# TrackieWay-OSS/TrackieLLM

Hardware: AMD Instinct MI355X
Metric: cortex cycles/sec (frame+1s audio+128 tok) (higher is better)
Workload: dtype int8 x q4_K/q6_K (i32 acc, f32 scales); 1 GPU; configs[3] fused cycle: YOLOv8n 640x640 frame (preprocess+network+NMS) + 1 s PCM (VAD + Whisper-tiny.en log-mel/encoder/16 forced decoder steps) + Mistral-7B Q4_K_M 64-token prefill and 128-token greedy decode, 3 concurrent HIP streams; concurrent_cycles_per_gpu=768, decode_groups=3, rows_per_llm_pass=256, layers=32, parallelism=replicas x1

## Files before the change

trackiellm_amd/csrc/audio/tk_audio_engine.h:

```cpp
#ifndef TK_AUDIO_ENGINE_H
#define TK_AUDIO_ENGINE_H

#include <hip/hip_runtime.h>
#include <stdint.h>

#include <string>
#include <vector>

#include "../common/tk_whisper_graph.h"

class TkWhisperModel {
public:
    TkWhisperHP hp{};
    TkWhManifest man;
    int device = 0;
    std::vector<float*> w;
    std::vector<uint8_t*> wt;
    bool prepare_tiles();
    int tensor_of(const float* dev_ptr) const;
    std::string error;
    ~TkWhisperModel();
    bool init(const TkWhisperHP& hp, int device);
    bool fill_synthetic(uint64_t seed);
    bool set_tensor(int idx, const float* host, size_t n);
    bool load_file(const char* path);
    bool load_ggml(class TkWhisperGgml& g);
};

class TkAsr {
public:
    TkWhisperModel* model = nullptr;
    int max_batch = 1;
    bool fast = false;
    std::string error;
    hipStream_t stream = nullptr;
    ~TkAsr();
    bool init(TkWhisperModel* m, int max_batch);
    bool transcribe(int B, const int16_t* pcm, int n_samples, const int32_t* prompt, int n_prompt, int n_steps, int32_t* tokens_out,
                    std::vector<float>* mel_out, std::vector<float>* enc_out, std::vector<float>* first_logits);
    bool transcribe_policy(int B, const int16_t* pcm, int n_samples, const int32_t* prompt, int n_prompt, int n_steps, float temperature, uint64_t seed,
                           int32_t* tokens_out, float* logprobs_out);
    bool transcribe_ref(int B, const int16_t* pcm, int n_samples, const int32_t* n_samples_row, const int32_t* prompt, int n_prompt, int n_steps, float temperature,
                        uint64_t seed, const uint8_t* suppress, int32_t token_beg, int32_t token_eot, int32_t* tokens_out, float* logprobs_out, int32_t* result_len,
                        int32_t* status);

private:
    friend struct TkAudioGpuOps;
    float* arena = nullptr;
    size_t arena_floats = 0, arena_used = 0;
    std::string launch_error;
    int16_t* pcm_dev = nullptr;
    size_t pcm_cap = 0;
    struct { bool on = false; float temp = 0.0f; uint64_t seed = 0; float* logprob = nullptr; int step = 0;
             bool filtered = false; int first_step = 0; const uint8_t* suppress = nullptr; int32_t* state = nullptr; int32_t beg = 0, eot = 0, tid0 = 0; } pick;
    uint8_t* suppress_dev = nullptr;
    std::vector<uint8_t> suppress_host;
    int32_t* wh_state = nullptr;
    float* lp_dev = nullptr;
    bool ensure_decode_buffers();
    std::vector<float> pick_logprobs;
};

class TkVadModel {
public:
    int device = 0, window = 480, hidden = 64;
    float *w1 = nullptr, *b1 = nullptr, *w2 = nullptr, *b2 = nullptr;
    float *x = nullptr, *hbuf = nullptr, *p = nullptr;
    int cap = 0;
    hipStream_t stream = nullptr;
    std::string error;
    ~TkVadModel();
    bool init(int device, int window, int hidden);
    bool fill_synthetic(uint64_t seed);
    bool infer(const float* windows_host, int n, float* prob_host);
};

#endif
```

trackiellm_amd/csrc/audio/tk_audio_engine.hip:

```cpp
#include "tk_audio_engine.h"
#include "tk_whisper_ggml.h"

#include <stdio.h>
#include <string.h>

#include "../nn/tk_gemm_tiled.h"
#include "../nn/tk_nn_kernels.h"

static inline hipError_t tk_create_perception_stream(hipStream_t* s) {
    int lo = 0, hi = 0;
    if (hipDeviceGetStreamPriorityRange(&lo, &hi) != hipSuccess) return hipStreamCreateWithFlags(s, hipStreamNonBlocking);
    return hipStreamCreateWithPriority(s, hipStreamNonBlocking, hi);
}

#define HIPQ(expr)                                                                              \
    do {                                                                                        \
        hipError_t e__ = (expr);                                                                \
        if (e__ != hipSuccess) {                                                                \
            char b__[256];                                                                      \
            snprintf(b__, sizeof b__, "%s failed: %s (%s:%d)", #expr, hipGetErrorString(e__), __FILE__, __LINE__); \
            error = b__;                                                                        \
            return false;                                                                       \
        }                                                                                       \
    } while (0)


__global__ void k_frames(const int16_t* pcm, int n_samples, int pcm_stride, int n_total, int T, const float* window, float* out) {
    const int b = blockIdx.z;
    const int64_t i = (int64_t)blockIdx.x * blockDim.x + threadIdx.x;
    if (i >= (int64_t)T * TK_WH_NFFT) return;
    const int t = (int)(i / TK_WH_NFFT), n = (int)(i % TK_WH_NFFT);
    int j = t * TK_WH_HOP + n - TK_WH_NFFT / 2;
    if (j < 0) j = -j;
    if (j >= n_total) j = 2 * (n_total - 1) - j;
    const float x = j < n_samples ? tk_divf((float)pcm[(int64_t)b * pcm_stride + j], 32768.0f) : 0.0f;
    out[((int64_t)b * T + t) * TK_WH_NFFT + n] = x * window[n];
}

__global__ void k_power(const float* ri, int64_t rows, int nb, float* out) {
    const int64_t i = (int64_t)blockIdx.x * blockDim.x + threadIdx.x;
    if (i >= rows * nb) return;
    const int64_t r = i / nb;
    const int f = (int)(i % nb);
    const float re = ri[r * 2 * nb + f], im = ri[r * 2 * nb + nb + f];
    out[i] = tk_fmaf(re, re, im * im);
}

__global__ __launch_bounds__(1024) void k_logmel_finish(float* mel, int per_b) {
    __shared__ float red[16];
    float* m = mel + (int64_t)blockIdx.x * per_b;
    float mx = -INFINITY;
    for (int i = threadIdx.x; i < per_b; i += 1024) {
        const float v = tk_log10f(tk_fmaxf(m[i], 1e-10f));
        m[i] = v;
        mx = tk_fmaxf(mx, v);
    }
    for (int s = 32; s >= 1; s >>= 1) mx = tk_fmaxf(mx, __shfl_xor(mx, s, 64));
    if ((threadIdx.x & 63) == 0) red[threadIdx.x >> 6] = mx;
    __syncthreads();
    mx = red[0];
    for (int w = 1; w < 16; ++w) mx = tk_fmaxf(mx, red[w]);
    const float floor_v = mx - 8.0f;
    for (int i = threadIdx.x; i < per_b; i += 1024) m[i] = (tk_fmaxf(m[i], floor_v) + 4.0f) * 0.25f;
}


#define TK_AT1_CK 64
#define TK_AT1_NS 3
__device__ __forceinline__ void at1_wait_vmcnt(int n) {
#define TK_VMW(k) case k: __builtin_amdgcn_s_waitcnt(0x0F70 | ((k) & 15) | (((k) >> 4) << 14)); break;
    switch (n) {
        TK_VMW(0) TK_VMW(1) TK_VMW(2) TK_VMW(3) TK_VMW(4) TK_VMW(5) TK_VMW(6) TK_VMW(7) TK_VMW(8) TK_VMW(9) TK_VMW(10) TK_VMW(11) TK_VMW(12)
        TK_VMW(13) TK_VMW(14) TK_VMW(15) TK_VMW(16)
        default: __builtin_amdgcn_s_waitcnt(0x0F70); break;
    }
#undef TK_VMW
}
__global__ __launch_bounds__(256) void k_attend1(const float* q, const float* k, const float* v, float* out, int Tk, int64_t q_bstride, int64_t kv_bstride, int d,
                                                 int hd, float scale, float* img ) {
    extern __shared__ __attribute__((aligned(16))) float att1_lds[];
    __shared__ float red[4];
    float* vring = att1_lds;
    float* sc = att1_lds + (size_t)TK_AT1_NS * TK_AT1_CK * hd;
    float* qs = sc + Tk;
    const int h = blockIdx.x, b = blockIdx.y, t0 = threadIdx.x, lane = t0 & 63;
    const int wave = __builtin_amdgcn_readfirstlane(t0 >> 6);
// ... 118 lines not shown
    float* image_for(const float* A, int M, int K, int lda) {
        pk.mark = a->arena_used;
        TkGemm g{};
        g.M = M; g.K = K;
        pk.img = raw_alloc(tk_tiled_gemm_scratch(g));
        pk.A = A; pk.M = M; pk.K = K; pk.lda = lda; pk.live = true;
        return pk.img;
    }
    void gemm(const TkGemm& g) {
        if (a->fast && long_ok) {
            drop_image();
            TkGemm f = g;
            f.fast = 1;
            tk_launch_gemm(f, s);
            return;
        }
        const int idx = tk_tiled_gemm_applies(g) ? a->model->tensor_of(g.B) : -1;
        if (idx < 0 || !a->model->wt[(size_t)idx]) { drop_image(); tk_launch_gemm(g, s); return; }
        if (!(pk.live && pk.A == g.A && pk.M == g.M && pk.K == g.K && pk.lda == g.lda)) {
            drop_image();
            pk.mark = a->arena_used;
            pk.img = raw_alloc(tk_tiled_gemm_scratch(g));
            tk_launch_pack_a(g.A, g.M, g.K, g.lda, 0, pk.img, s);
            pk.A = g.A; pk.M = g.M; pk.K = g.K; pk.lda = g.lda; pk.live = true;
        }
        const float* c0 = g.C;
        const float* c1 = g.C + (size_t)(g.M - 1) * g.ldc + g.N;
        const float* a0 = g.A;
        const float* a1 = g.A + (size_t)(g.M - 1) * g.lda + g.K;
        const bool in_place = c0 < a1 && a0 < c1;
        const bool plain = !g.residual && !g.c_feeds_linear && g.N % 16 == 0 && !in_place;
        if (plain) {
            if (pend.n > 0 && (pend.t.a_img != pk.img || pend.t.K != g.K || pend.t.nrows != g.M || pend.t.act != g.act)) flush();
            TkTiledGemm& t = pend.t;
            if (pend.n == 0) {
                t = TkTiledGemm{};
                t.wbytes = 4; t.K = g.K; t.ks = 1; t.nrows = g.M; t.slab_rows = 0; t.a_img = pk.img; t.a_ts = (size_t)g.K * 16;
                t.act = g.act; t.add_zero_bias = 1; t.per_seg = 1;
            }
            const int i = pend.n++;
            t.tiles[i] = a->model->wt[(size_t)idx]; t.row_tiles[i] = g.N / 16;
            t.seg_out[i] = g.C; t.seg_ldc[i] = g.ldc; t.seg_bias[i] = g.bias; t.seg_n[i] = g.N;
            if (pend.n == 3) flush();
            return;
        }
        flush();
        TkTiledGemm t{};
        t.tiles[0] = a->model->wt[(size_t)idx]; t.row_tiles[0] = (g.N + 15) / 16; t.nseg = 1; t.wbytes = 4;
        t.K = g.K; t.ks = 1; t.ldc = g.ldc; t.n_valid = g.N; t.nrows = g.M; t.slab_rows = 0;
        t.a_img = pk.img; t.a_ts = (size_t)g.K * 16; t.out = g.C;
        t.bias = g.bias; t.residual = g.residual; t.ldr = g.ldr; t.act = g.act; t.add_zero_bias = 1;
        const bool emit_img = g.c_feeds_linear && g.N % 128 == 0 && g.ldc == g.N && !g.residual && !in_place;
        float* cimg = nullptr;
        if (emit_img) {
            TkGemm nx{};
            nx.M = g.M; nx.K = g.N;
            cimg = raw_alloc(tk_tiled_gemm_scratch(nx));
            t.c_img = cimg;
        }
        if (!tk_launch_gemm_tiled(t, s)) tk_launch_gemm(g, s);
        if (emit_img) {
            pk.img = cimg; pk.A = g.C; pk.M = g.M; pk.K = g.N; pk.lda = g.ldc; pk.live = true;
            return;
        }
        if (in_place) drop_image();
    }
    void im2col1d(const float* x, int B, int T, int C, int ldx, int kw, int stride, int pad, float* col) { drop_image(); tk_launch_im2col1d(x, B, T, C, ldx, kw, stride, pad, col, s); }
    void layernorm(const float* x, int rows, int D, const float* w, const float* b, float* y) {
        drop_image();
        float* img = D % 128 == 0 && !(a->fast && long_ok) ? image_for(y, rows, D, D) : nullptr;
        tk_launch_layernorm(x, rows, D, w, b, TK_WH_LN_EPS, y, s, img);
    }
    void softmax_rows(float* x, int rows, int cols, int ld) { drop_image(); tk_launch_softmax_rows(x, rows, cols, ld, s); }
    bool attend1(const float* q, const float* k, const float* v, float* out, int B, int Tk, int64_t q_bstride, int64_t kv_bstride, int d, int nh) {
        drop_image();
        const int hd = d / nh;
        const size_t ldsb = ((size_t)TK_AT1_NS * TK_AT1_CK * hd + (size_t)Tk + (size_t)hd) * 4;
        if (hd > 256 || (hd & 15) || (d & 3) || Tk < 1 || ldsb > 60 * 1024) return false;
        float* img = (short_pass(B) && d % 128 == 0 && q_bstride == d) ? image_for(out, B, d, d) : nullptr;
        hipLaunchKernelGGL(k_attend1, dim3(nh, B), dim3(256), ldsb, s, q, k, v, out, Tk, q_bstride, kv_bstride, d, hd, tk_divf(1.0f, tk_sqrtf((float)hd)), img);
        return true;
    }
    bool attend_fused(const float* q, const float* k, const float* v, float* out, int B, int Tq, int Tk, int64_t q_bstride, int64_t kv_bstride, int d, int nh) {
        if (!a->fast || !long_ok || Tq < 2 || nh < 1 || d != nh * 64) return false;
        drop_image();
        return tk_launch_attention_h3(q, k, v, out, B, nh, Tq, Tk, q_bstride, kv_bstride, d, tk_divf(1.0f, tk_sqrtf(64.0f)), s);
    }
    void add_rows(float* x, const float* add, int rows, int D, int add_rows) { drop_image(); tk_launch_add_rows(x, add, rows, D, add_rows, s); }
    void embed_rows(const float* table, const float* pos, const int32_t* idx, const int32_t* pos_idx, int rows, int D, float* out) {
        drop_image();
        tk_launch_embed_rows(table, pos, idx, pos_idx, rows, D, out, s);
    }
    void argmax_rows(const float* x, int rows, int cols, int ld, int32_t* out) {
        drop_image();
        if (!a->pick.on) { tk_launch_argmax_rows(x, rows, cols, ld, out, s); return; }
        TkPick pk{a->pick.temp, a->pick.seed, (uint32_t)(a->pick.step * rows), a->pick.logprob ? a->pick.logprob + (size_t)a->pick.step * rows : nullptr};
        if (a->pick.filtered) {
            if (a->pick.step >= a->pick.first_step) {
                TkWhFilter f{a->pick.suppress, a->pick.state, a->pick.beg, a->pick.eot, a->pick.tid0};
                tk_launch_pick_rows_filtered(x, rows, cols, ld, out, pk, f, s);
            }
        } else {
            tk_launch_pick_rows(x, rows, cols, ld, out, pk, s);
        }
        a->pick.step++;
    }
    void frames(const int16_t* pcm, int B, int n_samples, int pcm_stride, int n_total, int T, const float* window, float* out) {
        drop_image();
        const int64_t per = (int64_t)T * TK_WH_NFFT;
        hipLaunchKernelGGL(k_frames, dim3((unsigned)((per + 255) / 256), 1, B), dim3(256), 0, s, pcm, n_samples, pcm_stride, n_total, T, window, out);
    }
    void power(const float* ri, int rows, int nb, float* out) {
        drop_image();
        const int64_t n = (int64_t)rows * nb;
        hipLaunchKernelGGL(k_power, dim3((unsigned)((n + 255) / 256)), dim3(256), 0, s, ri, (int64_t)rows, nb, out);
    }
    void logmel_finish(float* mel, int B, int per_b) { drop_image(); hipLaunchKernelGGL(k_logmel_finish, dim3(B), dim3(1024), 0, s, mel, per_b); }
};

struct TkAudioSizeOps {
    size_t used = 0, peak = 0;
    float* alloc(size_t n) { used += (n + 63) & ~(size_t)63; if (used > peak) peak = used; return nullptr; }
    int32_t* alloc_i32(size_t n) { return (int32_t*)alloc(n); }
    void gemm(const TkGemm& g) {
        if (!tk_tiled_gemm_applies(g)) return;
        size_t top = used + ((tk_tiled_gemm_scratch(g) + 63) & ~(size_t)63);
        if (g.c_feeds_linear) { TkGemm nx{}; nx.M = g.M; nx.K = g.N; top += (tk_tiled_gemm_scratch(nx) + 63) & ~(size_t)63; }
        if (top > peak) peak = top;
    }
    void image(int M, int K) {
        TkGemm g{};
        g.M = M; g.K = K;
        const size_t top = used + ((tk_tiled_gemm_scratch(g) + 63) & ~(size_t)63);
        if (top > peak) peak = top;
    }
    void im2col1d(const float*, int, int, int, int, int, int, int, float*) {}
    void layernorm(const float*, int rows, int D, const float*, const float*, float*) { image(rows, D); }
    void softmax_rows(float*, int, int, int) {}
    bool attend1(const float*, const float*, const float*, float*, int B, int, int64_t, int64_t, int d, int) { image(B, d); return true; }
    bool attend_fused(const float*, const float*, const float*, float*, int, int, int, int64_t, int64_t, int, int) { return false; }
    void add_rows(float*, const float*, int, int, int) {}
    void embed_rows(const float*, const float*, const int32_t*, const int32_t*, int, int, float*) {}
    void argmax_rows(const float*, int, int, int, int32_t*) {}
    void frames(const int16_t*, int, int, int, int, int, const float*, float*) {}
    void power(const float*, int, int, float*) {}
    void logmel_finish(float*, int, int) {}
};


TkWhisperModel::~TkWhisperModel() {
    (void)hipSetDevice(device);
    for (auto p : w) if (p) (void)hipFree(p);
    for (auto p : wt) if (p) (void)hipFree(p);
}

int TkWhisperModel::tensor_of(const float* dev_ptr) const {
    for (size_t i = 0; i < w.size(); ++i) if (w[i] == dev_ptr) return (int)i;
    return -1;
}

bool TkWhisperModel::prepare_tiles() {
    HIPQ(hipSetDevice(device));
    if (wt.size() != man.t.size()) wt.assign(man.t.size(), nullptr);
    for (size_t i = 0; i < man.t.size(); ++i) {
        const bool linear = man.t[i].kind == TK_WK_LINEAR_W || (int)i == man.tok_emb;
        if (!linear || man.t[i].cols % 128 || man.t[i].rows < 16 || wt[i]) continue;
        HIPQ(hipMalloc((void**)&wt[i], tk_tiled_weight_bytes(man.t[i].rows, man.t[i].cols, 4)));
        tk_launch_tile_weights(w[i], 4, man.t[i].rows, man.t[i].cols, wt[i], nullptr);
    }
// ... 22 lines not shown
        HIPQ(hipDeviceSynchronize());
    }
    return true;
}

bool TkWhisperModel::fill_synthetic(uint64_t seed) {
    std::vector<float> buf;
    for (size_t i = 0; i < man.t.size(); ++i) {
        buf.resize((size_t)man.t[i].rows * man.t[i].cols);
        tk_whisper_fill_tensor(hp, man, (int)i, seed, buf.data());
        if (!set_tensor((int)i, buf.data(), buf.size())) return false;
    }
    return true;
}

bool TkWhisperModel::load_file(const char* path) {
    FILE* f = fopen(path, "rb");
    if (!f) { error = std::string("cannot open ") + path; return false; }
    char magic[8];
    int32_t n = 0;
    bool ok = fread(magic, 1, 8, f) == 8 && memcmp(magic, "TKWHSP1", 8) == 0 && fread(&n, 4, 1, f) == 1 && n == (int)man.t.size();
    std::vector<float> buf;
    for (int i = 0; ok && i < n; ++i) {
        int64_t d[2];
        ok = fread(d, 8, 2, f) == 2;
        if (!ok) break;
        if (d[0] == 0) {
            buf.resize((size_t)man.t[i].rows * man.t[i].cols);
            tk_whisper_fill_tensor(hp, man, i, 0, buf.data());
        } else {
            ok = d[0] == man.t[i].rows && d[1] == man.t[i].cols;
            buf.resize((size_t)d[0] * d[1]);
            ok = ok && fread(buf.data(), 4, buf.size(), f) == buf.size();
        }
        ok = ok && set_tensor(i, buf.data(), buf.size());
    }
    fclose(f);
    if (!ok && error.empty()) error = "not a TKWHSP1 container for this geometry";
    return ok;
}

bool TkWhisperModel::load_ggml(TkWhisperGgml& g) {
    std::vector<float> buf;
    for (int i = 0; i < (int)man.t.size(); ++i) {
        bool found = false;
        if (!g.read(man, i, &buf, &found)) {
            if (found) { error = g.error; return false; }
            if (i != man.hann && i != man.dft) { error = "tensor " + man.t[i].name + " is missing from the checkpoint"; return false; }
            buf.resize((size_t)man.t[i].rows * man.t[i].cols);
            tk_whisper_fill_tensor(hp, man, i, 0, buf.data());
        }
        if (!set_tensor(i, buf.data(), buf.size())) return false;
    }
    return true;
}


TkAsr::~TkAsr() {
    if (model) (void)hipSetDevice(model->device);
    if (stream) (void)hipStreamSynchronize(stream);
    if (arena) (void)hipFree(arena);
    if (pcm_dev) (void)hipFree(pcm_dev);
    if (suppress_dev) (void)hipFree(suppress_dev);
    if (lp_dev) (void)hipFree(lp_dev);
    if (wh_state) (void)hipFree(wh_state);
    if (stream) (void)hipStreamDestroy(stream);
}

bool TkAsr::init(TkWhisperModel* m, int mb) {
    model = m;
    max_batch = mb;
    if (!m || mb < 1 || mb > 256) { error = "max_batch must be in [1,256]"; return false; }
    HIPQ(hipSetDevice(m->device));
    HIPQ(tk_create_perception_stream(&stream));
    TkAudioSizeOps so;
    std::vector<float*> nullw(m->man.t.size(), nullptr);
    TkWhisperGraph<TkAudioSizeOps> g{m->hp, m->man, nullw.data()};
    float* ml = g.mel(so, nullptr, mb, 0, 0);
    float* enc = g.encode(so, ml, mb);
    (void)g.begin_decode(so, enc, mb);
    arena_floats = so.peak + 4096 + (size_t)3 * m->hp.n_text_ctx * mb + 64;
    if (!m->prepare_tiles()) { error = m->error; return false; }
    if (!tk_gemm_tiled_prepare_device()) { error = "LDS opt-in of the tiled GEMM failed"; return false; }
    HIPQ(hipMalloc((void**)&arena, arena_floats * 4));
    return true;
}

bool TkAsr::transcribe_policy(int B, const int16_t* pcm, int n_samples, const int32_t* prompt, int n_prompt, int n_steps, float temperature, uint64_t seed,
                              int32_t* tokens_out, float* logprobs_out) {
    if (!(temperature >= 0.0f) || model->hp.n_vocab > 65536) { error = "temperature must be >= 0 and the vocabulary at most 65536 tokens"; return false; }
    const int total = n_prompt + n_steps - 1;
    if (B < 1 || total < 1) { error = "nothing to decode"; return false; }
    if (hipSetDevice(model->device) != hipSuccess) { error = "hipSetDevice failed"; return false; }
    if (!ensure_decode_buffers()) return false;
    if (total > model->hp.n_text_ctx || B > max_batch) { error = "prompt + steps exceed the text context"; return false; }
    float* d_lp = lp_dev;
    pick.on = true; pick.temp = temperature; pick.seed = seed; pick.logprob = d_lp; pick.step = 0;
    const bool ok = transcribe(B, pcm, n_samples, prompt, n_prompt, n_steps, tokens_out, nullptr, nullptr, nullptr);
    pick.on = false;
    bool copied = true;
    if (ok && logprobs_out) {
        pick_logprobs.resize((size_t)total * B);
        copied = hipMemcpyAsync(pick_logprobs.data(), d_lp, pick_logprobs.size() * sizeof(float), hipMemcpyDeviceToHost, stream) == hipSuccess &&
                 hipStreamSynchronize(stream) == hipSuccess;
        for (int step = 0; copied && step < n_steps; ++step)
            for (int b = 0; b < B; ++b) logprobs_out[(size_t)b * n_steps + step] = pick_logprobs[(size_t)(n_prompt - 1 + step) * B + b];
    }
    pick.logprob = nullptr;
    if (ok && !copied) error = "copy of the log-probabilities failed";
    return ok && copied;
}

bool TkAsr::ensure_decode_buffers() {
    const TkWhisperHP& h = model->hp;
    if (!lp_dev) HIPQ(hipMalloc((void**)&lp_dev, (size_t)max_batch * h.n_text_ctx * sizeof(float)));
    if (!suppress_dev) HIPQ(hipMalloc((void**)&suppress_dev, (size_t)h.n_vocab));
    if (!wh_state) HIPQ(hipMalloc((void**)&wh_state, (size_t)max_batch * TK_WH_STATE_INTS * sizeof(int32_t)));
    return true;
}

bool TkAsr::transcribe_ref(int B, const int16_t* pcm, int n_samples, const int32_t* n_samples_row, const int32_t* prompt, int n_prompt, int n_steps, float temperature,
                           uint64_t seed, const uint8_t* suppress, int32_t token_beg, int32_t token_eot, int32_t* tokens_out, float* logprobs_out, int32_t* result_len,
                           int32_t* status) {
    const TkWhisperHP& h = model->hp;
    if (!(temperature >= 0.0f) || h.n_vocab > 65536) { error = "temperature must be >= 0 and the vocabulary at most 65536 tokens"; return false; }
    if (B < 1 || B > max_batch || !suppress || !n_samples_row || token_beg <= token_eot || token_beg >= h.n_vocab) { error = "bad arguments to the reference-parameter decode"; return false; }
    const int total = n_prompt + n_steps - 1;
    if (total < 1) { error = "nothing to decode"; return false; }
    if (hipSetDevice(model->device) != hipSuccess) { error = "hipSetDevice failed"; return false; }
    if (!ensure_decode_buffers()) return false;
    if (total > h.n_text_ctx) { error = "prompt + steps exceed the text context"; return false; }
    if (suppress_host.size() != (size_t)h.n_vocab || memcmp(suppress_host.data(), suppress, (size_t)h.n_vocab) != 0) {
        HIPQ(hipStreamSynchronize(stream));
        suppress_host.assign(suppress, suppress + h.n_vocab);
        HIPQ(hipMemcpyAsync(suppress_dev, suppress_host.data(), (size_t)h.n_vocab, hipMemcpyHostToDevice, stream));
    }
    std::vector<int32_t> st0((size_t)B * TK_WH_STATE_INTS, 0);
    for (int b = 0; b < B; ++b) st0[(size_t)b * TK_WH_STATE_INTS + 7] = n_samples_row[b] / TK_WH_HOP;
    HIPQ(hipMemcpyAsync(wh_state, st0.data(), st0.size() * sizeof(int32_t), hipMemcpyHostToDevice, stream));
    float* d_lp = lp_dev;
    HIPQ(hipMemsetAsync(d_lp, 0, (size_t)total * B * sizeof(float), stream));
    pick.on = true; pick.temp = temperature; pick.seed = seed; pick.logprob = d_lp; pick.step = 0;
    pick.filtered = true; pick.first_step = n_prompt - 1; pick.suppress = suppress_dev; pick.state = wh_state; pick.beg = token_beg; pick.eot = token_eot;
    pick.tid0 = 50;
    const bool ok = transcribe(B, pcm, n_samples, prompt, n_prompt, n_steps, tokens_out, nullptr, nullptr, nullptr);
    pick.on = false; pick.filtered = false;
    bool copied = true;
    std::vector<int32_t> st1((size_t)B * TK_WH_STATE_INTS);
    if (ok) {
        pick_logprobs.resize((size_t)total * B);
        copied = hipMemcpyAsync(pick_logprobs.data(), d_lp, pick_logprobs.size() * sizeof(float), hipMemcpyDeviceToHost, stream) == hipSuccess &&
                 hipMemcpyAsync(st1.data(), wh_state, st1.size() * sizeof(int32_t), hipMemcpyDeviceToHost, stream) == hipSuccess &&
                 hipStreamSynchronize(stream) == hipSuccess;
        for (int b = 0; copied && b < B; ++b) {
            const int32_t* sb = &st1[(size_t)b * TK_WH_STATE_INTS];
            if (status) status[b] = sb[6];
            if (result_len) result_len[b] = sb[6] == 0 ? sb[0] : sb[5];
            for (int step = 0; logprobs_out && step < n_steps; ++step) logprobs_out[(size_t)b * n_steps + step] = pick_logprobs[(size_t)(n_prompt - 1 + step) * B + b];
        }
    }
    pick.logprob = nullptr;
    if (ok && !copied) error = "copy of the decode state failed";
    return ok && copied;
}

bool TkAsr::transcribe(int B, const int16_t* pcm, int n_samples, const int32_t* prompt, int n_prompt, int n_steps, int32_t* tokens_out,
// ... 140 lines not shown
```

trackiellm_amd/csrc/nn/tk_nn_kernels.h:

```cpp
#ifndef TK_NN_KERNELS_H
#define TK_NN_KERNELS_H

#include <hip/hip_runtime.h>
#include <stdint.h>

#include "../common/tk_gemm_desc.h"

void tk_launch_gemm(const TkGemm& g, hipStream_t s);
bool tk_gemm_im2col_ok(const float* x, int C, int ldx, const float* w);
bool tk_launch_conv_stem(const float* x, int B, int H, int W, int C, int ldx, const float* w, const float* bias, int act, int N, int k, int stride, int pad, float* y,
                         int ldy, hipStream_t s);
bool tk_nn_prepare_device();
bool tk_launch_attention_h3(const float* q, const float* k, const float* v, float* out, int B, int nh, int Tq, int Tk, int64_t q_bstride, int64_t kv_bstride, int d,
                            float scale, hipStream_t s);

void tk_launch_im2col(const float* x, int B, int H, int W, int C, int ldx, int kh, int kw, int stride, int pad, float* col, hipStream_t s);
void tk_launch_maxpool5(const float* x, int B, int H, int W, int C, int ldx, float* y, int ldy, hipStream_t s);
void tk_launch_upsample2x(const float* x, int B, int H, int W, int C, int ldx, float* y, int ldy, hipStream_t s);
void tk_launch_copy_cols(const float* x, int rows, int C, int ldx, float* y, int ldy, hipStream_t s);
void tk_launch_im2col1d(const float* x, int B, int T, int C, int ldx, int kw, int stride, int pad, float* col, hipStream_t s);
void tk_launch_embed_rows(const float* table, const float* pos, const int32_t* idx, const int32_t* pos_idx, int rows, int D, float* out, hipStream_t s);
void tk_launch_argmax_rows(const float* x, int rows, int cols, int ld, int32_t* out, hipStream_t s);
struct TkPick { float temp; uint64_t seed; uint32_t counter0; float* logprob; };
void tk_launch_pick_rows(const float* x, int rows, int cols, int ld, int32_t* out, const TkPick& pk, hipStream_t s);
#define TK_WH_STATE_INTS 8
struct TkWhFilter { const uint8_t* suppress; int32_t* state; int32_t beg, eot, tid0; };
void tk_launch_pick_rows_filtered(const float* x, int rows, int cols, int ld, int32_t* out, const TkPick& pk, const TkWhFilter& f, hipStream_t s);
void tk_launch_layernorm(const float* x, int rows, int D, const float* w, const float* b, float eps, float* y, hipStream_t s, float* img = nullptr );
void tk_launch_softmax_rows(float* x, int rows, int cols, int ld, hipStream_t s);
void tk_launch_add_rows(float* x, const float* add, int rows, int D, int add_rows, hipStream_t s);

#endif
```

trackiellm_amd/csrc/nn/tk_nn_kernels.hip:

```cpp
#include "tk_nn_kernels.h"

#include <atomic>
#include <mutex>

#include "../common/tk_exact_math.h"
#include "../common/tk_sample_device.h"

typedef float v16f __attribute__((ext_vector_type(16)));

#define BM 64
#define BN 64
#define BK 32
#define LDS_LD (BK + 1)

__device__ __forceinline__ float ldb1(const float* B, int f16, int64_t i) {
    return f16 ? (float)((const _Float16*)B)[i] : B[i];
}
__device__ __forceinline__ void ldb4(const float* B, int f16, int64_t i, float* out) {
    if (f16) {
        const uint2 t = *(const uint2*)((const _Float16*)B + i);
        const _Float16* h = (const _Float16*)&t;
        out[0] = (float)h[0]; out[1] = (float)h[1]; out[2] = (float)h[2]; out[3] = (float)h[3];
    } else {
        const float4 t = *(const float4*)(B + i);
// ... 619 lines not shown
        }
        *(v8h*)(Vh + vd * FA_VLD + vc * 8) = hi;
        *(v8h*)(Vl + vd * FA_VLD + vc * 8) = lo;
    };
    const float L2E = 1.4426950408889634f;
    gload(0);
    for (int k0 = 0; k0 < Tk; k0 += 32) {
        __syncthreads();
        lstore();
        __syncthreads();
        if (k0 + 32 < Tk) gload(k0 + 32);
        v16f s_hh, s_hx;
#pragma unroll
        for (int r = 0; r < 16; ++r) { s_hh[r] = 0.0f; s_hx[r] = 0.0f; }
#pragma unroll
        for (int ks = 0; ks < 4; ++ks) {
            const v8h ah = *(const v8h*)(Kh + n * FA_KLD + ks * 16 + g * 8), al = *(const v8h*)(Kl + n * FA_KLD + ks * 16 + g * 8);
            s_hh = H3_MFMA(ah, qh[ks], s_hh);
            s_hx = H3_MFMA(ah, ql[ks], s_hx);
            s_hx = H3_MFMA(al, qh[ks], s_hx);
        }
        float st[16], mloc = -INFINITY;
#pragma unroll
        for (int r = 0; r < 16; ++r) {
            const int key = k0 + 4 * g + (r & 3) + 8 * (r >> 2);
            st[r] = key < Tk ? s_hh[r] + s_hx[r] * (1.0f / H3_SCALE) : -INFINITY;
            mloc = fmaxf(mloc, st[r]);
        }
        mloc = fmaxf(mloc, __shfl_xor(mloc, 32));
        const float m_new = fmaxf(m_run, mloc);
        const float alpha = __builtin_amdgcn_exp2f((m_run - m_new) * L2E);
        m_run = m_new;
        float psum = 0.0f;
        v8h ph[2], pl[2];
#pragma unroll
        for (int r = 0; r < 16; ++r) {
            const float pr = __builtin_amdgcn_exp2f((st[r] - m_new) * L2E);
            psum += pr;
            const _Float16 hi = (_Float16)pr;
            ph[r >> 3][r & 7] = hi;
            pl[r >> 3][r & 7] = (_Float16)((pr - (float)hi) * H3_SCALE);
        }
        l_run = l_run * alpha + psum;
        if (__builtin_amdgcn_ballot_w64(alpha != 1.0f)) {
#pragma unroll
            for (int t = 0; t < 2; ++t)
#pragma unroll
                for (int r = 0; r < 16; ++r) { o_hh[t][r] *= alpha; o_hx[t][r] *= alpha; }
        }
#pragma unroll
        for (int t = 0; t < 2; ++t)
#pragma unroll
            for (int sp = 0; sp < 2; ++sp) {
                const v8h vh = *(const v8h*)(Vh + (t * 32 + n) * FA_VLD + sp * 16 + g * 8), vl = *(const v8h*)(Vl + (t * 32 + n) * FA_VLD + sp * 16 + g * 8);
                o_hh[t] = H3_MFMA(vh, ph[sp], o_hh[t]);
                o_hx[t] = H3_MFMA(vh, pl[sp], o_hx[t]);
                o_hx[t] = H3_MFMA(vl, ph[sp], o_hx[t]);
            }
    }
    const float l = l_run + __shfl_xor(l_run, 32);
    if (qrow >= Tq) return;
    const float inv = __builtin_amdgcn_rcpf(l);
    float* op = out + (int64_t)b * q_bstride + (int64_t)qrow * d + (int64_t)head * 64;
#pragma unroll
    for (int t = 0; t < 2; ++t)
#pragma unroll
        for (int rr = 0; rr < 4; ++rr) {
            float4 w;
            w.x = (o_hh[t][4 * rr + 0] + o_hx[t][4 * rr + 0] * (1.0f / H3_SCALE)) * inv;
            w.y = (o_hh[t][4 * rr + 1] + o_hx[t][4 * rr + 1] * (1.0f / H3_SCALE)) * inv;
            w.z = (o_hh[t][4 * rr + 2] + o_hx[t][4 * rr + 2] * (1.0f / H3_SCALE)) * inv;
            w.w = (o_hh[t][4 * rr + 3] + o_hx[t][4 * rr + 3] * (1.0f / H3_SCALE)) * inv;
            *(float4*)(op + t * 32 + 4 * g + 8 * rr) = w;
        }
}

bool tk_launch_attention_h3(const float* q, const float* k, const float* v, float* out, int B, int nh, int Tq, int Tk, int64_t q_bstride, int64_t kv_bstride, int d,
                            float scale, hipStream_t s) {
    if (d != nh * 64 || (d & 3) || Tq < 1 || Tk < 1 || ((((uintptr_t)q) | ((uintptr_t)k) | ((uintptr_t)v) | ((uintptr_t)out)) & 15) || (q_bstride & 3) || (kv_bstride & 3)) return false;
    hipLaunchKernelGGL(k_attention_h3, dim3((Tq + 127) / 128, nh, B), dim3(256), 0, s, q, k, v, out, Tq, Tk, q_bstride, kv_bstride, d, scale);
    return true;
}

static std::atomic<bool> g_big_opted[64];
static std::mutex g_big_mu;
bool tk_nn_prepare_device() {
    const size_t lds = (size_t)2 * (LBM + LBN) * LDS_LD * sizeof(float);
    int dev = 0;
    if (hipGetDevice(&dev) != hipSuccess || dev < 0 || dev >= 64) return false;
    if (g_big_opted[dev].load(std::memory_order_acquire)) return true;
    std::lock_guard<std::mutex> lk(g_big_mu);
    const void* fns[4] = {(const void*)k_gemm_f32_big<false, 0>, (const void*)k_gemm_f32_big<false, 1>, (const void*)k_gemm_f32_big<false, 2>,
                          (const void*)k_gemm_f32_big<true, 1>};
    for (const void* f : fns)
        if (hipFuncSetAttribute(f, hipFuncAttributeMaxDynamicSharedMemorySize, (int)lds) != hipSuccess) return false;
    const void* h3[2] = {(const void*)k_gemm_h3_big<false>, (const void*)k_gemm_h3_big<true>};
    for (const void* f : h3)
        if (hipFuncSetAttribute(f, hipFuncAttributeMaxDynamicSharedMemorySize, (int)H3_BIG_LDS) != hipSuccess) return false;
    g_big_opted[dev].store(true, std::memory_order_release);
    return true;
}

static bool tk_gemm_fast(const TkGemm& g) {
    auto m4 = [](int64_t v) { return (v & 3) == 0; };
    if (g.b_f16 || !m4(g.K) || !m4(g.ldb) || (((uintptr_t)g.B) & 15)) return false;
    if (g.im_C == 0 && (!m4(g.lda) || (((uintptr_t)g.A) & 15))) return false;
    if (g.b_kn && !m4(g.N)) return false;
    if (g.batch > 1 && (!m4(g.sA) || !m4(g.sB))) return false;
    if (g.batch_inner > 0 && (!m4(g.sA2) || !m4(g.sB2))) return false;
    return true;
}

void tk_launch_gemm(const TkGemm& g, hipStream_t s) {
    const int nz = g.batch > 0 ? g.batch : 1;
    const bool im = g.im_C > 0;
    const int path = tk_gemm_fast(g) ? (g.b_kn ? 2 : 1) : 0;
#define TK_GEMM_PATHS(KERNEL, GRID, LDS)                                                                      \
    do {                                                                                                      \
        if (im) hipLaunchKernelGGL((KERNEL<true, 1>), GRID, dim3(256), LDS, s, g);                            \
        else if (path == 1) hipLaunchKernelGGL((KERNEL<false, 1>), GRID, dim3(256), LDS, s, g);               \
        else if (path == 2) hipLaunchKernelGGL((KERNEL<false, 2>), GRID, dim3(256), LDS, s, g);               \
        else hipLaunchKernelGGL((KERNEL<false, 0>), GRID, dim3(256), LDS, s, g);                              \
    } while (0)
    const bool fast = g.fast != 0 && !g.b_kn && (im || path == 1);
    if (fast && g.N >= 96) {
        (void)tk_nn_prepare_device();
        const dim3 grid((g.N + LBN - 1) / LBN, (g.M + LBM - 1) / LBM, nz);
        if (im) hipLaunchKernelGGL((k_gemm_h3_big<true>), grid, dim3(256), H3_BIG_LDS, s, g);
        else hipLaunchKernelGGL((k_gemm_h3_big<false>), grid, dim3(256), H3_BIG_LDS, s, g);
        return;
    }
    if (fast && nz == 1 && g.batch_inner == 0) {
        const dim3 grid(1, (g.M + NBM - 1) / NBM, 1);
        const int nt = (g.N + 31) / 32;
#define TK_TALL_H3(NTV)                                                                                       \
    do {                                                                                                      \
        if (im) hipLaunchKernelGGL((k_gemm_h3_tall<true, NTV>), grid, dim3(256), 0, s, g);                    \
        else hipLaunchKernelGGL((k_gemm_h3_tall<false, NTV>), grid, dim3(256), 0, s, g);                      \
    } while (0)
        if (nt == 1) TK_TALL_H3(1); else if (nt == 2) TK_TALL_H3(2); else TK_TALL_H3(3);
#undef TK_TALL_H3
        return;
    }
    if (g.M >= 256 && g.N >= 96) {
        const size_t lds = (size_t)2 * (LBM + LBN) * LDS_LD * sizeof(float);
        (void)tk_nn_prepare_device();
        const dim3 grid((g.N + LBN - 1) / LBN, (g.M + LBM - 1) / LBM, nz);
        TK_GEMM_PATHS(k_gemm_f32_big, grid, lds);
        return;
    }
    if (g.N < 96 && g.M >= 4 * NBM && !g.b_kn && !g.b_f16 && nz == 1 && g.batch_inner == 0) {
        const dim3 grid(1, (g.M + NBM - 1) / NBM, 1);
        const int nt = (g.N + 31) / 32;
#define TK_TALL(NTV)                                                                                          \
    do {                                                                                                      \
        if (im) hipLaunchKernelGGL((k_gemm_f32_tall<true, 1, NTV>), grid, dim3(256), 0, s, g);                \
        else if (path == 1) hipLaunchKernelGGL((k_gemm_f32_tall<false, 1, NTV>), grid, dim3(256), 0, s, g);   \
        else hipLaunchKernelGGL((k_gemm_f32_tall<false, 0, NTV>), grid, dim3(256), 0, s, g);                  \
    } while (0)
        if (nt == 1) TK_TALL(1); else if (nt == 2) TK_TALL(2); else TK_TALL(3);
#undef TK_TALL
        return;
    }
    const dim3 grid((g.N + BN - 1) / BN, (g.M + BM - 1) / BM, nz);
    TK_GEMM_PATHS(k_gemm_f32, grid, 0);
#undef TK_GEMM_PATHS
}

bool tk_gemm_im2col_ok(const float* x, int C, int ldx, const float* w) {
    return C > 0 && (C & 3) == 0 && (ldx & 3) == 0 && ((((uintptr_t)x) | ((uintptr_t)w)) & 15) == 0;
}

template <int N, int C, int KW>
__global__ __launch_bounds__(256) void k_conv_stem(const float* x, int H, int W, int ldx, const float* w, const float* bias, int act, int stride, int pad, int Ho,
                                                   int Wo, uint32_t total, float* y, int ldy) {
    constexpr int K = KW * KW * C;
    __shared__ __attribute__((aligned(16))) float ws[K * N];
    for (int i = threadIdx.x; i < K * N; i += 256) ws[i] = w[(i % N) * K + i / N];
    __syncthreads();
    const uint32_t t = blockIdx.x * 256u + threadIdx.x;
    if (t >= total) return;
    const uint32_t ox = t % (uint32_t)Wo, r = t / (uint32_t)Wo, oy = r % (uint32_t)Ho, b = r / (uint32_t)Ho;
// ... 507 lines not shown
```

Measured before the change: 185.1 cycles/s.

## Add exact fused MFMA attention kernel for Whisper non-fast path

Adds a new fused attention kernel that computes QK^T with fp32 MFMA, keeps the score rows in LDS for an exact softmax, and multiplies by V with MFMA. Whisper ASR in exact (non-fast) mode now uses it instead of the separate GEMM, softmax and GEMM launches. The goal is to cut kernel launches and the global-memory round trips of the score matrix. It needs up to 128KB of LDS per block, which can lower occupancy, and an environment variable restores the unfused path.

```diff
diff --git a/trackiellm_amd/csrc/audio/tk_audio_engine.h b/trackiellm_amd/csrc/audio/tk_audio_engine.h
--- a/trackiellm_amd/csrc/audio/tk_audio_engine.h
+++ b/trackiellm_amd/csrc/audio/tk_audio_engine.h
@@ -32,6 +32,7 @@
     TkWhisperModel* model = nullptr;
     int max_batch = 1;
     bool fast = false;
+    bool unfused_attention = false;
     std::string error;
     hipStream_t stream = nullptr;
     ~TkAsr();
diff --git a/trackiellm_amd/csrc/audio/tk_audio_engine.hip b/trackiellm_amd/csrc/audio/tk_audio_engine.hip
--- a/trackiellm_amd/csrc/audio/tk_audio_engine.hip
+++ b/trackiellm_amd/csrc/audio/tk_audio_engine.hip
@@ -2,6 +2,7 @@
 #include "tk_whisper_ggml.h"
 
 #include <stdio.h>
+#include <stdlib.h>
 #include <string.h>
 
 #include "../nn/tk_gemm_tiled.h"
@@ -286,9 +287,14 @@
         return true;
     }
     bool attend_fused(const float* q, const float* k, const float* v, float* out, int B, int Tq, int Tk, int64_t q_bstride, int64_t kv_bstride, int d, int nh) {
-        if (!a->fast || !long_ok || Tq < 2 || nh < 1 || d != nh * 64) return false;
+        if (a->fast && long_ok) {
+            if (Tq < 2 || nh < 1 || d != nh * 64) return false;
+            drop_image();
+            return tk_launch_attention_h3(q, k, v, out, B, nh, Tq, Tk, q_bstride, kv_bstride, d, tk_divf(1.0f, tk_sqrtf(64.0f)), s);
+        }
+        if (a->unfused_attention || Tq < 2 || nh < 1 || d % nh) return false;
         drop_image();
-        return tk_launch_attention_h3(q, k, v, out, B, nh, Tq, Tk, q_bstride, kv_bstride, d, tk_divf(1.0f, tk_sqrtf(64.0f)), s);
+        return tk_launch_attention_exact(q, k, v, out, B, nh, Tq, Tk, q_bstride, kv_bstride, d, tk_divf(1.0f, tk_sqrtf((float)(d / nh))), s);
     }
     void add_rows(float* x, const float* add, int rows, int D, int add_rows) { drop_image(); tk_launch_add_rows(x, add, rows, D, add_rows, s); }
     void embed_rows(const float* table, const float* pos, const int32_t* idx, const int32_t* pos_idx, int rows, int D, float* out) {
@@ -477,6 +483,9 @@
     arena_floats = so.peak + 4096 + (size_t)3 * m->hp.n_text_ctx * mb + 64;
     if (!m->prepare_tiles()) { error = m->error; return false; }
     if (!tk_gemm_tiled_prepare_device()) { error = "LDS opt-in of the tiled GEMM failed"; return false; }
+    if (!tk_nn_prepare_device()) { error = "LDS opt-in of the large-tile GEMM and the fused attention failed"; return false; }
+    const char* att = getenv("TK_MI355X_ASR_ATTENTION");
+    unfused_attention = att && strcmp(att, "unfused") == 0;
     HIPQ(hipMalloc((void**)&arena, arena_floats * 4));
     return true;
 }
diff --git a/trackiellm_amd/csrc/nn/tk_nn_kernels.h b/trackiellm_amd/csrc/nn/tk_nn_kernels.h
--- a/trackiellm_amd/csrc/nn/tk_nn_kernels.h
+++ b/trackiellm_amd/csrc/nn/tk_nn_kernels.h
@@ -13,6 +13,8 @@
 bool tk_nn_prepare_device();
 bool tk_launch_attention_h3(const float* q, const float* k, const float* v, float* out, int B, int nh, int Tq, int Tk, int64_t q_bstride, int64_t kv_bstride, int d,
                             float scale, hipStream_t s);
+bool tk_launch_attention_exact(const float* q, const float* k, const float* v, float* out, int B, int nh, int Tq, int Tk, int64_t q_bstride, int64_t kv_bstride, int d,
+                               float alpha, hipStream_t s);
 
 void tk_launch_im2col(const float* x, int B, int H, int W, int C, int ldx, int kh, int kw, int stride, int pad, float* col, hipStream_t s);
 void tk_launch_maxpool5(const float* x, int B, int H, int W, int C, int ldx, float* y, int ldy, hipStream_t s);
diff --git a/trackiellm_amd/csrc/nn/tk_nn_kernels.hip b/trackiellm_amd/csrc/nn/tk_nn_kernels.hip
--- a/trackiellm_amd/csrc/nn/tk_nn_kernels.hip
+++ b/trackiellm_amd/csrc/nn/tk_nn_kernels.hip
@@ -725,6 +725,186 @@
     return true;
 }
 
+typedef float v4f __attribute__((ext_vector_type(4)));
+#define AX_ROWS 16
+#define AX_WAVES 8
+#define AX_KLD 17
+#define AX_CH 32
+#define AX_LDS_MAX (128 * 1024)
+static inline int ax_pitch(int Tk) { return ((Tk + 1) & ~3) + 2; }
+static inline size_t ax_lds_bytes(int Tk, int hd) { return ((size_t)AX_ROWS * ax_pitch(Tk) + (size_t)AX_WAVES * hd * AX_KLD) * sizeof(float); }
+
+template <int HD>
+__global__ __launch_bounds__(64 * AX_WAVES) void k_attention_exact(const float* __restrict__ q, const float* __restrict__ k, const float* __restrict__ v, float* __restrict__ out,
+                                                                  int Tq, int Tk, int64_t q_bstride, int64_t kv_bstride, int d, float alpha, int pitch) {
+    extern __shared__ __attribute__((aligned(16))) float ax_lds[];
+    float* S = ax_lds;
+    const int tid = threadIdx.x, lane = tid & 63, n = lane & 15, g = lane >> 4;
+    const int wave = __builtin_amdgcn_readfirstlane(tid >> 6);
+    float* Ks = ax_lds + AX_ROWS * pitch + wave * (HD * AX_KLD);
+    const int head = blockIdx.y, b = blockIdx.z, row0 = blockIdx.x * AX_ROWS;
+    const float* qp = q + (int64_t)b * q_bstride + (int64_t)head * HD;
+    const float* kp = k + (int64_t)b * kv_bstride + (int64_t)head * HD;
+    const float* vp = v + (int64_t)b * kv_bstride + (int64_t)head * HD;
+
+    {
+        float qa[HD / 4];
+#pragma unroll
+        for (int s = 0; s < HD / 4; ++s) {
+            const float t = qp[(int64_t)(row0 + n < Tq ? row0 + n : Tq - 1) * d + 4 * s + g];
+            qa[s] = row0 + n < Tq ? t : 0.0f;
+        }
+        constexpr int GPK = HD / 4, NV = HD / 16;
+        const int ntiles = (Tk + 15) >> 4;
+        float rk[NV][4];
+        auto kload = [&](int kt) {
+#pragma unroll
+            for (int i = 0; i < NV; ++i) {
+                const int e = lane + 64 * i, key = kt * 16 + e / GPK;
+                const float4 t = *(const float4*)(kp + (int64_t)(key < Tk ? key : Tk - 1) * d + (e % GPK) * 4);
+                rk[i][0] = t.x; rk[i][1] = t.y; rk[i][2] = t.z; rk[i][3] = t.w;
+            }
+        };
+        if (wave < ntiles) kload(wave);
+        for (int kt = wave; kt < ntiles; kt += AX_WAVES) {
+#pragma unroll
+            for (int i = 0; i < NV; ++i) {
+                const int e = lane + 64 * i, kk = e / GPK, c = e % GPK;
+                const bool ok = kt * 16 + kk < Tk;
+#pragma unroll
+                for (int j = 0; j < 4; ++j) Ks[(4 * c + j) * AX_KLD + kk] = ok ? rk[i][j] : 0.0f;
+            }
+            if (kt + AX_WAVES < ntiles) kload(kt + AX_WAVES);
+            __builtin_amdgcn_wave_barrier();
+            v4f acc = {0.0f, 0.0f, 0.0f, 0.0f};
+#pragma unroll
+            for (int s = 0; s < HD / 4; ++s) acc = __builtin_amdgcn_mfma_f32_16x16x4f32(qa[s], Ks[(4 * s + g) * AX_KLD + n], acc, 0, 0, 0);
+            __builtin_amdgcn_wave_barrier();
+            const int key = kt * 16 + n;
+            if (key < Tk) {
+#pragma unroll
+                for (int r = 0; r < 4; ++r) {
+                    float x = acc[r];
+                    if (alpha != 1.0f) x = x * alpha;
+                    S[(4 * g + r) * pitch + key] = x + 0.0f;
+                }
+            }
+        }
+    }
+    __syncthreads();
+
+    const int rows = Tq - row0 < AX_ROWS ? Tq - row0 : AX_ROWS;
+    for (int r = wave; r < rows; r += AX_WAVES) {
+        float* sr = S + r * pitch;
+        float m = -INFINITY;
+        for (int i0 = lane; i0 < Tk + lane; i0 += 256) {
+#pragma unroll
+            for (int qq = 0; qq < 4; ++qq) {
+                const int i = i0 + 64 * qq;
+                m = tk_fmaxf(m, sr[i < Tk ? i : Tk - 1]);
+            }
+        }
+        for (int s = 32; s >= 1; s >>= 1) m = tk_fmaxf(m, __shfl_xor(m, s, 64));
+        float p[4] = {0.0f, 0.0f, 0.0f, 0.0f};
+        for (int i0 = lane; i0 < Tk + lane; i0 += 256) {
+            float e[4];
+#pragma unroll
+            for (int qq = 0; qq < 4; ++qq) {
+                const int i = i0 + 64 * qq;
+                e[qq] = tk_expf(sr[i < Tk ? i : Tk - 1] - m);
+            }
+            __builtin_amdgcn_wave_barrier();
+#pragma unroll
+            for (int qq = 0; qq < 4; ++qq) {
+                const int i = i0 + 64 * qq;
+                if (i < Tk) { sr[i] = e[qq]; p[qq] = p[qq] + e[qq]; }
+            }
+        }
+        for (int s = 32; s >= 1; s >>= 1) {
+#pragma unroll
+            for (int qq = 0; qq < 4; ++qq) p[qq] = p[qq] + __shfl_xor(p[qq], s, 64);
+        }
+        const float tot = ((p[0] + p[1]) + p[2]) + p[3];
+        for (int i0 = lane; i0 < Tk + lane; i0 += 256) {
+            float e[4];
+#pragma unroll
+            for (int qq = 0; qq < 4; ++qq) {
+                const int i = i0 + 64 * qq;
+                e[qq] = tk_divf(sr[i < Tk ? i : Tk - 1], tot);
+            }
+            __builtin_amdgcn_wave_barrier();
+#pragma unroll
+            for (int qq = 0; qq < 4; ++qq) {
+                const int i = i0 + 64 * qq;
+                if (i < Tk) sr[i] = e[qq];
+            }
+        }
+    }
+    __syncthreads();
+
+    if (wave * 16 >= HD) return;
+    const float* sp = S + n * pitch + g;
+    const float* vc = vp + (int64_t)g * d + wave * 16 + n;
+    const int nwhole = Tk / (4 * AX_CH), tail0 = nwhole * (4 * AX_CH);
+    float vt[AX_CH], vb[2][AX_CH];
+    if (tail0 < Tk) {
+#pragma unroll
+        for (int i = 0; i < AX_CH; ++i) {
+            const int j = tail0 + 4 * i + g;
+            vt[i] = vp[(int64_t)(j < Tk ? j : Tk - 1) * d + wave * 16 + n];
+        }
+    }
+    __builtin_amdgcn_sched_barrier(0);
+    auto vload = [&](int c, float* dst) {
+        const float* src = vc + (int64_t)(c < nwhole ? c : nwhole - 1) * (4 * AX_CH) * d;
+#pragma unroll
+        for (int i = 0; i < AX_CH; ++i) dst[i] = src[(int64_t)(4 * i) * d];
+    };
+    v4f acc = {0.0f, 0.0f, 0.0f, 0.0f};
+    auto chain = [&](int c, const float* vbuf) {
+        const float* src = sp + c * (4 * AX_CH);
+        float a[AX_CH];
+#pragma unroll
+        for (int i = 0; i < AX_CH; ++i) a[i] = src[4 * i];
+#pragma unroll
+        for (int i = 0; i < AX_CH; ++i) acc = __builtin_amdgcn_mfma_f32_16x16x4f32(a[i], vbuf[i], acc, 0, 0, 0);
+    };
+    if (nwhole > 0) {
+        vload(0, vb[0]);
+        for (int c = 0; c + 1 < nwhole; c += 2) {
+            vload(c + 1, vb[1]);
+            __builtin_amdgcn_sched_barrier(0);
+            chain(c, vb[0]);
+            __builtin_amdgcn_sched_barrier(0);
+            vload(c + 2, vb[0]);
+            __builtin_amdgcn_sched_barrier(0);
+            chain(c + 1, vb[1]);
+            __builtin_amdgcn_sched_barrier(0);
+        }
+        if (nwhole & 1) chain(nwhole - 1, vb[0]);
+    }
+    __builtin_amdgcn_sched_barrier(0);
+    if (tail0 < Tk) {
+        float a[AX_CH];
+#pragma unroll
+        for (int i = 0; i < AX_CH; ++i) {
+            const int j = tail0 + 4 * i + g;
+            const float t = S[n * pitch + (j < Tk ? j : Tk - 1)];
+            a[i] = j < Tk ? t : 0.0f;
+        }
+#pragma unroll
+        for (int i = 0; i < AX_CH; ++i)
+            if (tail0 + 4 * i < Tk)
+                acc = __builtin_amdgcn_mfma_f32_16x16x4f32(a[i], tail0 + 4 * i + g < Tk ? vt[i] : 0.0f, acc, 0, 0, 0);
+    }
+    float* op = out + (int64_t)b * q_bstride + (int64_t)head * HD + wave * 16 + n;
+#pragma unroll
+    for (int r = 0; r < 4; ++r) {
+        const int row = row0 + 4 * g + r;
+        if (row < Tq) op[(int64_t)row * d] = acc[r] + 0.0f;
+    }
+}
+
 static std::atomic<bool> g_big_opted[64];
 static std::mutex g_big_mu;
 bool tk_nn_prepare_device() {
@@ -740,7 +920,24 @@
     const void* h3[2] = {(const void*)k_gemm_h3_big<false>, (const void*)k_gemm_h3_big<true>};
     for (const void* f : h3)
         if (hipFuncSetAttribute(f, hipFuncAttributeMaxDynamicSharedMemorySize, (int)H3_BIG_LDS) != hipSuccess) return false;
+    const void* ax[2] = {(const void*)k_attention_exact<64>, (const void*)k_attention_exact<32>};
+    for (const void* f : ax)
+        if (hipFuncSetAttribute(f, hipFuncAttributeMaxDynamicSharedMemorySize, AX_LDS_MAX) != hipSuccess) return false;
     g_big_opted[dev].store(true, std::memory_order_release);
+    return true;
+}
+
+bool tk_launch_attention_exact(const float* q, const float* k, const float* v, float* out, int B, int nh, int Tq, int Tk, int64_t q_bstride, int64_t kv_bstride, int d,
+                               float alpha, hipStream_t s) {
+    if (nh < 1 || d % nh || Tq < 2 || Tk < 1 || B < 1 || B > 65535 || nh > 65535) return false;
+    const int hd = d / nh;
+    if ((hd != 64 && hd != 32) || ax_lds_bytes(Tk, hd) > AX_LDS_MAX) return false;
+    if ((d & 3) || (kv_bstride & 3) || (((uintptr_t)k) & 15)) return false;
+    if (!tk_nn_prepare_device()) return false;
+    const dim3 grid((Tq + AX_ROWS - 1) / AX_ROWS, nh, B);
+    const size_t lds = ax_lds_bytes(Tk, hd);
+    if (hd == 64) hipLaunchKernelGGL(k_attention_exact<64>, grid, dim3(64 * AX_WAVES), lds, s, q, k, v, out, Tq, Tk, q_bstride, kv_bstride, d, alpha, ax_pitch(Tk));
+    else hipLaunchKernelGGL(k_attention_exact<32>, grid, dim3(64 * AX_WAVES), lds, s, q, k, v, out, Tq, Tk, q_bstride, kv_bstride, d, alpha, ax_pitch(Tk));
     return true;
 }
 
```

After: 182.6 cycles/s. 1.3% lower.
